# jgkellymit/GENIE-SMEM

Measured on AMD Instinct MI355X. Metric: query-bases/sec SMEM discovery, 100kb ref x 150bp reads; bit-exact SMEM set, higher is better.
Workload: dtype u8/int32 (2-bit packed bases, int32 SA rows; f64 only in the RMI predict)

## Files before the change

### genie-smem_amd/csrc/kernels.hip

```cpp
#include <hip/hip_runtime.h>

#include <algorithm>
#include <cstdio>
#include <cstdlib>
#include <mutex>
#include <string>

#include "genie_internal.h"

namespace genie {

namespace {

constexpr int kWave = 64;

__device__ __forceinline__ int rfl(int v) { return __builtin_amdgcn_readfirstlane(v); }
__device__ __forceinline__ void set_wave_priority(int i)
{
    switch (i & 3) {
    case 0: __builtin_amdgcn_s_setprio(0); break;
    case 1: __builtin_amdgcn_s_setprio(1); break;
    case 2: __builtin_amdgcn_s_setprio(2); break;
    default: __builtin_amdgcn_s_setprio(3); break;
    }
}

__device__ __forceinline__ void scalar_touch_lines(const void *p, uint32_t bytes)
{
    uint32_t d, off;
    asm volatile("s_mov_b32 %[off], 0\n"
                 "1:\n\t"
                 "s_load_dword %[d], %[p], %[off]\n\t"
                 "s_add_u32 %[off], %[off], 64\n\t"
                 "s_cmp_lt_u32 %[off], %[n]\n\t"
                 "s_cbranch_scc1 1b\n\t"
                 "s_waitcnt lgkmcnt(0)"
                 : [d] "=&s"(d), [off] "=&s"(off)
                 : [p] "s"(reinterpret_cast<uint64_t>(p) & ~3ull), [n] "s"(bytes)
                 : "scc", "memory");
}

__device__ __forceinline__ void wave_lds_fence()
{
    __builtin_amdgcn_fence(__ATOMIC_ACQ_REL, "wavefront");
    __builtin_amdgcn_wave_barrier();
}

__device__ __forceinline__ uint64_t funnel(uint64_t w0, uint64_t w1, int sh )
{
    return sh ? (w0 << sh) | (w1 >> (64 - sh)) : w0;
}

__device__ __forceinline__ uint64_t qwin(const uint64_t *qp, int pos)
{
    int i = pos >> 5;
    return funnel(qp[i], qp[i + 1], (pos & 31) * 2);
}

__device__ __forceinline__ uint64_t rwin(const RefRec *ref, int pos)
{
    const ulonglong2 v = *reinterpret_cast<const ulonglong2 *>(ref + (pos >> 5));
    return funnel(v.x, v.y, (pos & 31) * 2);
}

struct QWords {
    const uint64_t *p;
    __device__ __forceinline__ uint64_t win(int pos) const { return qwin(p, pos); }
};
struct QRecs {
    const RefRec *p;
    __device__ __forceinline__ uint64_t win(int pos) const { return rwin(p, pos); }
};
struct QPlain {
    const uint64_t *p;
    __device__ __forceinline__ uint64_t win(int pos) const
    {
        typedef uint64_t u64x2 __attribute__((ext_vector_type(2)));
        typedef u64x2 u64x2_a8 __attribute__((aligned(8)));
        const u64x2 v = *reinterpret_cast<const u64x2_a8 *>(p + (pos >> 5));
        return funnel(v.x, v.y, (pos & 31) * 2);
    }
};

template <class D>
__device__ __forceinline__ uint32_t dir_lb(const DevIndex &ix, const D dir, uint32_t code, int m)
{
    const uint32_t x = code << (2 * (ix.P - m));
    uint32_t v = dir[x];
#pragma unroll
    for (int l = 0; l < GENIE_MAX_DIR_BITS; l++)
        if (l >= m && l < ix.P && ix.padtail[l] == x) v--;
    return v;
}

template <class D>
__device__ __forceinline__ uint32_t dir_ub(const DevIndex &ix, const D dir, uint32_t code, int m)
{
    const uint32_t x = (code + 1) << (2 * (ix.P - m));
    uint32_t v = dir[x];
#pragma unroll
    for (int l = 1; l < GENIE_MAX_DIR_BITS; l++)
        if (l < ix.P && ix.padtail[l] == x) v--;
    return v;
}

struct Cmp {
    int l;
    bool less;
};

template <class Q>
__device__ __forceinline__ Cmp cmp_suffix(const DevIndex &ix, const Q qp, int a, int m, int s, int skip)
{
    const int avail = ix.n - s;
    const int lim = m < avail ? m : avail;
    int l = skip;
    bool less = false;
    bool diff = false;
    while (l < lim) {
        const uint64_t xq = qp.win(a + l), xr = rwin(ix.ref, s + l);
        const uint64_t x = xq ^ xr;
        if (x) {
            l += __clzll((long long)x) >> 1;
            less = xr < xq;
            diff = true;
            break;
        }
        l += 32;
    }
    if (!diff || l >= lim) {
        l = lim;
        less = lim < m;
    }
    return {l, less};
}

template <class Q>
__device__ __forceinline__ Cmp cmp_rec(const DevIndex &ix, const Q qp, int a, int m, const SaRec rec, uint64_t xq)
{
    const int avail = ix.n - rec.s;
    const int lim = m < avail ? m : avail;
    int l = ix.P;
    bool less;
    const uint64_t x = xq ^ rec.key;
    if (x) {
        l += __clzll((long long)x) >> 1;
        less = rec.key < xq;
        if (l >= lim) { l = lim; less = lim < m; }
    } else if (l + 32 >= lim) {
        l = lim;
        less = lim < m;
    } else {
        return cmp_suffix(ix, qp, a, m, rec.s, l + 32);
    }
    return {l, less};
}

__device__ __forceinline__ int pick_probe(int lo, int hi, uint32_t xq32, uint32_t vlo, uint32_t vhi, int step)
{
    const int n = hi - lo;
    if ((step & 1) || n <= 2 || vhi <= vlo) return (lo + hi) >> 1;
    if (xq32 <= vlo) return lo;
    if (xq32 >= vhi) return hi - 1;
    const float f = (float)(xq32 - vlo) / (float)(vhi - vlo);
    int mid = lo + (int)(f * (float)n);
    mid = mid < lo ? lo : (mid > hi - 1 ? hi - 1 : mid);
    return mid;
}

typedef uint32_t nt_u4 __attribute__((ext_vector_type(4)));
typedef nt_u4 nt_u4_unaligned __attribute__((aligned(1)));
__device__ __forceinline__ void store_nt(void *dst, uint4 v)
{
    __builtin_nontemporal_store(nt_u4{v.x, v.y, v.z, v.w}, reinterpret_cast<nt_u4 *>(dst));
}

__device__ __forceinline__ SaRec load_rec(const SaRec *sa, int row)
{
    int4 v = *reinterpret_cast<const int4 *>(sa + row);
    asm volatile("" : "+v"(v.x), "+v"(v.y), "+v"(v.z), "+v"(v.w));
    SaRec r;
    r.s = v.x;
    r.pad = 0;
    r.key = ((uint64_t)(uint32_t)v.w << 32) | (uint32_t)v.z;
    return r;
}

__device__ __forceinline__ bool lut_probe(const DevIndex &ix, uint32_t code, int &lo, int &hi)
{
    uint32_t p = (uint32_t)(((uint64_t)(code * 0x9E3779B1u) * (uint64_t)ix.lut_slots) >> 32);
    for (uint32_t tries = 0; tries < ix.lut_slots; tries++) {
        const int4 v = *reinterpret_cast<const int4 *>(ix.lut + p);
        if (v.y < 0) return false;
        if ((uint32_t)v.x == code) { lo = v.y; hi = v.z; return true; }
        p = p + 1 == ix.lut_slots ? 0 : p + 1;
    }
    return false;
}

__device__ __forceinline__ double rmi_predict(const DevIndex &ix, const RmiModel *leaf, int leaf_cnt, uint32_t code,
                                              int *leaf_idx = nullptr)
{
    const double x = (double)code;
    double p = 0.0;
    int idx = 0;
    for (int l = 0; l < ix.nlev; l++) {
        if (leaf_idx && l == ix.nlev - 1) *leaf_idx = idx;
        double2 m;
        if (leaf && l == ix.nlev - 1 && idx < leaf_cnt) m = *reinterpret_cast<const double2 *>(leaf + idx);
        else m = *reinterpret_cast<const double2 *>(ix.rmi + ix.rmi_off[l] + idx);
        p = __dadd_rn(__dmul_rn(m.x, x), m.y);
        const int scale = ix.rmi_scale[l];
        idx = !(p > 0.0) ? 0 : (p >= (double)scale ? scale - 1 : (int)p);
    }
    return p;
}

__device__ __forceinline__ int kmer_cmp_row(const DevIndex &ix, int r, uint32_t code)
{
    const int s = ix.sa[r].s;
    const int avail = ix.n - s;
    if (avail == 0) return -1;
    const uint64_t w = rwin(ix.ref, s);
    if (avail >= ix.K) {
        const uint32_t rc = (uint32_t)(w >> (64 - 2 * ix.K));
        return rc < code ? -1 : (rc > code ? 1 : 0);
    }
    const uint32_t rc = (uint32_t)(w >> (64 - 2 * avail));
    const uint32_t qc = code >> (2 * (ix.K - avail));
    return rc <= qc ? -1 : 1;
}

__device__ __forceinline__ bool rmi_lookup(const DevIndex &ix, const RmiModel *leaf, uint32_t code, int &lo, int &hi,
                                           double *pred_out)
{
    int leaf_idx = 0;
    const double p = rmi_predict(ix, leaf, 0, code, &leaf_idx);
    if (pred_out) *pred_out = p;
    const int rows = ix.n + 1;
    const int r0 = !(p > 0.0) ? 0 : (p >= (double)rows ? rows - 1 : (int)p);
    int L, R;
    bool fenced = false;
    if (ix.rmi_err) {
        const int e = ix.rmi_err[leaf_idx];
        L = r0 - e < 0 ? 0 : r0 - e;
        R = r0 + e + 1 > rows ? rows : r0 + e + 1;
        int l2 = L, r2 = R;
        while (l2 < r2) {
            const int mid = (l2 + r2) >> 1;
            if (kmer_cmp_row(ix, mid, code) < 0) l2 = mid + 1; else r2 = mid;
        }
        if (l2 < rows && kmer_cmp_row(ix, l2, code) == 0 && (l2 > L || L == 0 || kmer_cmp_row(ix, l2 - 1, code) < 0)) {
            L = R = l2;
            fenced = true;
        }
    }
    if (!fenced) {
    if (kmer_cmp_row(ix, r0, code) < 0) {
        L = r0 + 1;
        R = rows;
        for (int step = 1;; step <<= 1) {
            const int pr = r0 + step;
            if (pr >= rows) break;
            if (kmer_cmp_row(ix, pr, code) < 0) L = pr + 1;
            else { R = pr; break; }
        }
    } else {
        R = r0;
        L = 0;
        for (int step = 1;; step <<= 1) {
            const int pr = r0 - step;
            if (pr < 0) break;
            if (kmer_cmp_row(ix, pr, code) < 0) { L = pr + 1; break; }
            R = pr;
        }
    }
    }
    while (L < R) {
        const int mid = (L + R) >> 1;
        if (kmer_cmp_row(ix, mid, code) < 0) L = mid + 1; else R = mid;
    }
    const int first = L;
    if (first >= rows || kmer_cmp_row(ix, first, code) != 0) { lo = first; hi = first - 1; return false; }
    int a = first, b = rows;
    for (int step = 1;; step <<= 1) {
        const int pr = first + step;
        if (pr >= rows) break;
        if (kmer_cmp_row(ix, pr, code) == 0) a = pr;
        else { b = pr; break; }
    }
    while (b - a > 1) {
        const int mid = (a + b) >> 1;
        if (kmer_cmp_row(ix, mid, code) == 0) a = mid; else b = mid;
    }
    lo = first;
    hi = a;
    return true;
}

template <class Q>
__device__ __forceinline__ int2 sa_interval(const DevIndex &ix, const uint32_t *dir, const Q qp, int a, int m)
{
    if (m == 0) return make_int2(0, ix.n);
    const int P = ix.P;
    const uint64_t w = qp.win(a);
    if (m <= P) {
        const uint32_t code = (uint32_t)(w >> (64 - 2 * m));
        const int lb = (int)dir_lb(ix, dir, code, m), ub = (int)dir_ub(ix, dir, code, m);
        return lb < ub ? make_int2(lb, ub - 1) : make_int2(-1, -1);
    }
    const uint64_t xq = qp.win(a + P);
    int lo, hi, h;
    int known = -1;
    if (ix.P2 && m >= ix.P2) {
        int4 hd = *reinterpret_cast<const int4 *>(ix.dir2 + (uint32_t)(w >> (64 - 2 * ix.P2)));
        asm volatile("" : "+v"(hd.x), "+v"(hd.y), "+v"(hd.z), "+v"(hd.w));
        const uint32_t cnt = (uint32_t)hd.y & ~kHeadShort;
        if (cnt == 0) return make_int2(-1, -1);
        lo = hd.x;
        hi = h = hd.x + (int)cnt;
        const uint64_t key = ((uint64_t)(uint32_t)hd.w << 32) | (uint32_t)hd.z;
        const uint64_t x = xq ^ key;
        if (!((uint32_t)hd.y & kHeadShort) && (x != 0 || m <= P + 32)) {
            const int l = x ? P + (__clzll((long long)x) >> 1) : m;
            if (l >= m) { h = lo; known = lo; }
            else if (key < xq) lo = lo + 1;
            else h = lo;
        }
    } else {
        const uint32_t b = (uint32_t)(w >> (64 - 2 * P));
        lo = (int)dir[b];
        hi = h = (int)dir_ub(ix, dir, b, P);
    }
    uint32_t vlo = 0, vhi = 0xFFFFFFFFu;
    int step = 0;
    while (lo < h) {
        const int mid = pick_probe(lo, h, (uint32_t)(xq >> 32), vlo, vhi, step++);
        const SaRec rec = load_rec(ix.sa, mid);
        const Cmp c = cmp_rec(ix, qp, a, m, rec, xq);
        if (c.less) { lo = mid + 1; vlo = (uint32_t)(rec.key >> 32); }
        else { h = mid; vhi = (uint32_t)(rec.key >> 32); known = c.l >= m ? mid : -1; }
    }
    const int first = lo;
    if (known == first) lo = first + 1;
    h = hi;
    int stepw = 1;
    while (lo < h) {
        int mid = stepw ? lo + stepw - 1 : (lo + h) >> 1;
        if (mid >= h) mid = (lo + h) >> 1;
        if (cmp_rec(ix, qp, a, m, load_rec(ix.sa, mid), xq).l >= m) { lo = mid + 1; stepw = stepw && stepw < (1 << 20) ? stepw << 1 : stepw; }
        else { h = mid; stepw = 0; }
    }
    return first < lo ? make_int2(first, lo - 1) : make_int2(-1, -1);
}

struct WaveScratch {
    uint64_t *qp;
    uint8_t *raw;
};

__host__ __device__ inline int scratch_qp_bytes(int Lmax) { return (((Lmax + 31) / 32 + 2) * 8 + 15) & ~15; }
__host__ __device__ inline int scratch_raw_bytes(int Lmax) { return (Lmax + 15) & ~15; }
__host__ __device__ inline int scratch_bytes(int Lmax) { return scratch_qp_bytes(Lmax) + scratch_raw_bytes(Lmax); }

__device__ __forceinline__ WaveScratch carve(uint8_t *base, int Lmax)
{
    WaveScratch s;
    s.qp = reinterpret_cast<uint64_t *>(base);
    s.raw = base + scratch_qp_bytes(Lmax);
    return s;
}

__device__ __forceinline__ bool load_and_pack(const uint8_t *src, int L, int Lmax, const WaveScratch &ws, int lane)
{
    uint8_t *raw = ws.raw;
    bool bad = false;
    for (int i = lane; i < L; i += kWave) {
        const uint8_t c = src[i];
        bad |= c > 3;
        raw[i] = c;
    }
    wave_lds_fence();
// ... 792 lines not shown
```

### genie-smem_amd/csrc/short_read_kernel.inc

```

template <bool WIDE>
struct ReadTraits {
    typedef uint8_t fwd_t;
    static constexpr int kj_bits = 16, kj_shift = 8;
};
template <>
struct ReadTraits<true> {
    typedef uint16_t fwd_t;
    static constexpr int kj_bits = 32, kj_shift = 16;
};


typedef unsigned short kb_us2 __attribute__((ext_vector_type(2)));
__device__ __forceinline__ uint32_t kb_pk_max(uint32_t a, uint32_t b)
{
    return __builtin_bit_cast(uint32_t, __builtin_elementwise_max(__builtin_bit_cast(kb_us2, a), __builtin_bit_cast(kb_us2, b)));
}

constexpr int kPairHeadWords = 4;

__device__ __forceinline__ int block_exclusive_scan(int v, int &total)
{
    __shared__ int wave_total[16];
    const int lane = threadIdx.x & (kWave - 1), wave = threadIdx.x >> 6;
// ... 25 lines not shown
                                                        uint8_t *__restrict__ counts8, uint8_t *__restrict__ status8)
{
    extern __shared__ __align__(16) uint8_t smem[];
    typedef ReadTraits<false>::fwd_t fwd_t;
    constexpr int kBits = ReadTraits<false>::kj_bits, kShift = ReadTraits<false>::kj_shift, kPer = 64 / kBits;
    const long long r0 = (long long)blockIdx.x * blockDim.x;
    {
        const int rows = (int)(N - r0 < (long long)blockDim.x ? N - r0 : (long long)blockDim.x);
        const uint4 *src = reinterpret_cast<const uint4 *>(reinterpret_cast<const uint8_t *>(fwd_in) + r0 * (long long)fwd_stride);
        uint32_t *dst = reinterpret_cast<uint32_t *>(smem);
        const int ldw = fwd_lds >> 2, upr = fwd_stride >> 4;
        const uint32_t recip = (uint32_t)((0x100000000ull + (uint64_t)upr - 1) / (uint64_t)upr);
        const int units = rows * upr;
        constexpr int kInFlight = 8;
        for (int e0 = threadIdx.x; e0 < units; e0 += kInFlight * blockDim.x) {
            uint4 v[kInFlight];
#pragma unroll
            for (int u = 0; u < kInFlight; u++) {
                const int e = e0 + u * blockDim.x;
                v[u] = e < units ? src[e] : make_uint4(0, 0, 0, 0);
            }
#pragma unroll
            for (int u = 0; u < kInFlight; u++) {
                const int e = e0 + u * blockDim.x;
                if (e < units) {
                    const int row = upr > 1 ? (int)__umulhi((uint32_t)e, recip) : e;
                    const int col = 4 * (e - row * upr);
                    uint32_t *d = dst + row * ldw + col;
                    d[0] = v[u].x;
                    if (col + 1 < ldw) d[1] = v[u].y;
                    if (col + 2 < ldw) d[2] = v[u].z;
                    if (col + 3 < ldw) d[3] = v[u].w;
                }
            }
        }
        __syncthreads();
    }
    const long long r = r0 + threadIdx.x;
    const bool valid = r < N;
    int cnt = 0;
    if (valid) {
        int st = status[r];
        const int L = lens ? lens[r] : fixed_len;
        const fwd_t *fw = reinterpret_cast<const fwd_t *>(smem + threadIdx.x * fwd_lds);
        unsigned long long *out64 = reinterpret_cast<unsigned long long *>(reinterpret_cast<uint8_t *>(kj_out) +
                                                                           r * (long long)kj_stride * (kBits / 8));
        unsigned long long *head64 = reinterpret_cast<unsigned long long *>(head_out + r * (long long)head_stride);
        unsigned long long acc = 0, acc0 = 0;

#define EMIT(kk, jj)                                                          \
        do {                                                                      \
            const int s_ = cnt + 1;                                               \
            const unsigned long long v_ = (unsigned long long)(uint32_t)((kk) | ((jj) << kShift)) << (kBits * (s_ & (kPer - 1))); \
            if (s_ < kPer) acc0 |= v_;                                            \
            else {                                                                \
                acc |= v_;                                                        \
                if ((s_ & (kPer - 1)) == kPer - 1) { (s_ / kPer < kPairHeadWords ? head64 : out64)[s_ / kPer] = acc; acc = 0; } \
            }                                                                     \
            cnt++;                                                                \
        } while (0)

        if (st == GENIE_READ_OK && L > 0) {
            int i = 0, kprev = -1;
            const uint32_t *fw32 = reinterpret_cast<const uint32_t *>(fw);
            while (i < L) {
                const int p0 = kprev + 1;
                const uint32_t i4 = (uint32_t)i * 0x01010101u;
                int sd = p0 >> 2;
                uint32_t x = (fw32[sd] ^ i4) & (~0u << (8 * (p0 & 3)));
                while (x == 0 && sd < (i >> 2)) x = fw32[++sd] ^ i4;
                const int s0 = 4 * sd + ((__ffs((int)x) - 1) >> 3);
                if (x == 0 || s0 > i) { st = GENIE_READ_ABSENT_BASE; break; }
                const uint32_t *pd = fw32 + (s0 >> 2);
                int more = (i >> 2) - (s0 >> 2);
                uint32_t pos = (uint32_t)(s0 >> 2) * 0x04040404u + 0x03020100u;
                uint32_t vb = ~0u << (8 * (s0 & 3));
                const uint32_t vl = ~0u >> (8 * (3 - (i & 3)));
                if (more == 0) vb &= vl;
                uint32_t len4 = (*pd - pos) & vb, pin4 = ~pos & vb;
                uint32_t top0 = __builtin_amdgcn_perm(len4, pin4, 0x05010400u), top1 = __builtin_amdgcn_perm(len4, pin4, 0x07030602u);
                if (more > 0) {
                    while (--more > 0) {
                        pos += 0x04040404u;
                        len4 = *++pd - pos;
                        pin4 = ~pos;
                        top0 = kb_pk_max(top0, __builtin_amdgcn_perm(len4, pin4, 0x05010400u));
                        top1 = kb_pk_max(top1, __builtin_amdgcn_perm(len4, pin4, 0x07030602u));
                    }
                    pos += 0x04040404u;
                    len4 = (*++pd - pos) & vl;
                    pin4 = ~pos & vl;
                    top0 = kb_pk_max(top0, __builtin_amdgcn_perm(len4, pin4, 0x05010400u));
                    top1 = kb_pk_max(top1, __builtin_amdgcn_perm(len4, pin4, 0x07030602u));
                }
                const uint32_t mx = kb_pk_max(top0, top1);
                const uint32_t key = max(mx & 0xFFFFu, mx >> 16);
                const int best = (int)(key >> 8), bk = 255 - (int)(key & 255u);
                if (best == 0) { st = GENIE_READ_ABSENT_BASE; break; }
                if (MODE != GENIE_MODE_BWA || best >= min_len) EMIT(bk, bk + best);
                i = bk + best;
                kprev = bk;
            }
            if (st != GENIE_READ_OK) cnt = 0;
            else {
                if (cnt + 1 >= kPer && ((cnt + 1) & (kPer - 1))) ((cnt + 1) / kPer < kPairHeadWords ? head64 : out64)[(cnt + 1) / kPer] = acc;
                if (cnt > cap) st = GENIE_READ_OVERFLOW;
            }
        }
#undef EMIT
        head64[0] = cnt ? acc0 | (unsigned long long)(uint32_t)cnt : 0ull;
        status[r] = st;
        if (counts8) {
            counts8[r] = (uint8_t)cnt;
            status8[r] = (uint8_t)st;
        }
    }
    if (block_sums) {
        int total;
        const int before = block_exclusive_scan(cnt, total);
        if (valid) counts[r] = before;
        if (threadIdx.x == 0) block_sums[blockIdx.x] = (unsigned long long)total;
    } else if (valid) {
        counts[r] = cnt;
    }
}

template <int G>
__device__ __forceinline__ uint32_t group_max(uint32_t v)
{
    v = max(v, (uint32_t)__builtin_amdgcn_update_dpp(0, (int)v, 0xB1, 0xf, 0xf, true));
    if (G >= 4) v = max(v, (uint32_t)__builtin_amdgcn_update_dpp(0, (int)v, 0x4E, 0xf, 0xf, true));
    if (G >= 8) v = max(v, (uint32_t)__builtin_amdgcn_update_dpp(0, (int)v, 0x141, 0xf, 0xf, true));
    if (G == 16) v = max(v, (uint32_t)__builtin_amdgcn_update_dpp(0, (int)v, 0x140, 0xf, 0xf, true));
    return v;
}

constexpr int kLongWin = 128;
constexpr int kLongRowBytes = 2 * kLongWin + 16;
template <int MODE, int G, int V = 1>
__global__ void __launch_bounds__(256) traverse_long_kernel(const int32_t *__restrict__ lens, long long N, int fixed_len, int min_len,
                                                             const uint8_t *__restrict__ fwd_in, int fwd_stride,
                                                             int32_t *__restrict__ counts, uint32_t *__restrict__ kj_out,
                                                             int kj_stride, int cap, int32_t *__restrict__ status,
                                                             unsigned long long *__restrict__ block_sums)
{
    static_assert((V == 1 && (G == 8 || G == 16)) || (V == 8 && (G == 2 || G == 4)), "lanes per read / positions per lane");
    extern __shared__ __align__(16) uint8_t smem[];
    uint8_t *wrow = smem + (threadIdx.x / G) * kLongRowBytes;
    const int row_chunks = fwd_stride >> 4;
    int wb = -(1 << 20);
    constexpr int kShift = ReadTraits<true>::kj_shift;
    const int lane = threadIdx.x & (kWave - 1), sub = lane & (G - 1);
    const long long r = (long long)blockIdx.x * (blockDim.x / G) + (threadIdx.x / G);
    const bool valid = r < N;
    int st = valid ? status[r] : GENIE_READ_OK;
    const int L = valid ? (lens ? lens[r] : fixed_len) : 0;
    const uint16_t *fw = reinterpret_cast<const uint16_t *>(fwd_in + (valid ? r : 0) * (long long)fwd_stride);
    uint32_t *row = kj_out + (valid ? r : 0) * (long long)kj_stride;
    int i = 0, cnt = 0;
    uint32_t mine = 0;
    bool go = valid && st == GENIE_READ_OK && L > 0;
    int kprev = -1;
    while (__any(go)) {
        uint32_t best = 0;
        int top = i;
        bool more = go;
        if (V == 8) {
            int ctop = i >> 3;
            const uint32_t reach = ((uint32_t)i << 16) | 0xFFFFu;
            bool first = true;
            const int need_lo = (kprev + 1) & ~7;
            const bool fits = go && i - need_lo < kLongWin;
            const bool reload = fits && !(need_lo >= wb && i < wb + kLongWin);
            if (__any(reload)) {
                if (reload) {
                    wb = need_lo;
                    uint4 t[kLongWin / 8 / G];
#pragma unroll
                    for (int u = 0; u < kLongWin / 8 / G; u++) {
                        const int c = (wb >> 3) + sub + G * u;
                        t[u] = c < row_chunks ? *reinterpret_cast<const uint4 *>(fw + 8 * c) : make_uint4(0, 0, 0, 0);
                    }
#pragma unroll
                    for (int u = 0; u < kLongWin / 8 / G; u++) *reinterpret_cast<uint4 *>(wrow + 16 * (sub + G * u)) = t[u];
                }
                wave_lds_fence();
            }
            while (__any(more)) {
                const int c = ctop - sub;
                const bool inb = more && c >= 0;
                uint4 q = make_uint4(0, 0, 0, 0);
                if (inb) {
                    if (fits && 8 * c >= wb) q = *reinterpret_cast<const uint4 *>(wrow + 2 * (8 * c - wb));
                    else q = *reinterpret_cast<const uint4 *>(fw + 8 * c);
                }
                uint32_t qd[4] = {q.x, q.y, q.z, q.w};
                if (first) {
                    const int jmax = (sub == 0) ? (i & 7) : 7;
#pragma unroll
                    for (int d = 0; d < 4; d++) qd[d] &= jmax >= 2 * d + 1 ? 0xFFFFFFFFu : (jmax >= 2 * d ? 0x0000FFFFu : 0u);
                    first = false;
                }
                const uint32_t c0 = (uint32_t)(0xFFFF - 8 * c) - ((uint32_t)(8 * c) << 16);
                uint32_t kmax = 0;
#pragma unroll
                for (int j = 0; j < 8; j++) {
                    const uint32_t vh = (j & 1) ? (qd[j >> 1] & 0xFFFF0000u) : (qd[j >> 1] << 16);
                    const uint32_t key = vh > reach ? vh + (c0 - (uint32_t)j * 0x10001u) : 0u;
                    kmax = max(kmax, key);
                }
                best = max(best, group_max<G>(kmax));
                const bool low = inb && (qd[0] << 16) > reach;
                ctop -= G;
                more = more && ((__ballot(low) >> (lane | (G - 1))) & 1ull);
            }
        }
        while (V == 1 && __any(more)) {
            const int k = top - sub;
            const bool in = more && k > kprev;
            const int v = in ? (int)fw[k] : 0;
            const bool covers = in && v > i;
            const uint32_t key = covers ? ((uint32_t)(v - k) << 16) | (uint32_t)(0xFFFF - k) : 0u;
            best = max(best, group_max<G>(key));
            top -= G;
            more = more && ((__ballot(covers) >> (lane | (G - 1))) & 1ull);
        }
        if (go) {
            const int blen = (int)(best >> 16), bk = 0xFFFF - (int)(best & 0xFFFFu);
            if (blen == 0) { st = GENIE_READ_ABSENT_BASE; go = false; }
            else {
                if (MODE != GENIE_MODE_BWA || blen >= min_len) {
                    const int s_ = cnt + 1;
                    if (sub == (s_ & (G - 1))) mine = (uint32_t)(bk | ((bk + blen) << kShift));
                    if ((s_ & (G - 1)) == G - 1) {
                        const int idx = (s_ & ~(G - 1)) + sub;
                        if (idx > 0) row[idx] = mine;
                    }
                    cnt++;
                }
                kprev = bk;
                i = bk + blen;
                go = i < L;
            }
        }
    }
    if (valid) {
        if (st != GENIE_READ_OK) cnt = 0;
        else {
            const int idx = ((cnt + 1) & ~(G - 1)) + sub;
            if (((cnt + 1) & (G - 1)) != 0 && idx >= 1 && idx <= cnt) row[idx] = mine;
            if (cnt > cap) st = GENIE_READ_OVERFLOW;
        }
        if (sub == 0) {
            row[0] = (uint32_t)cnt;
            status[r] = st;
        }
    }
    if (block_sums) {
        int total;
        const int before = block_exclusive_scan(valid && sub == 0 ? cnt : 0, total);
        if (valid && sub == 0) counts[r] = before;
        if (threadIdx.x == 0) block_sums[blockIdx.x] = (unsigned long long)total;
    } else if (valid && sub == 0) {
        counts[r] = cnt;
    }
}

constexpr int kIvWaves = 8;
constexpr int kIvUnroll = 1;
constexpr int kIvList = 128;

struct RowEscapes {
    unsigned long long *count;
    long long *list;
    long long cap;
};
template <int COUT>
__device__ __forceinline__ void emit_row(void *out, long long idx, int k, int j, int lo, int hi, const RowEscapes &esc)
{
    if (COUT == 0) {
        store_nt(reinterpret_cast<int4 *>(out) + idx, make_uint4((uint32_t)k, (uint32_t)j, (uint32_t)lo, (uint32_t)hi));
        return;
    }
    constexpr uint32_t kTop = COUT == 1 ? 0xFFFFu : 0xFFu;
    uint32_t span = (uint32_t)(hi - lo);
    if (span >= kTop) {
        const unsigned long long slot = atomicAdd(esc.count, 1ull);
        if ((long long)slot < esc.cap) {
            esc.list[2 * slot] = idx;
            esc.list[2 * slot + 1] = hi;
        }
        span = kTop;
    }
    if (COUT == 1) {
        reinterpret_cast<uint2 *>(out)[idx] = make_uint2((uint32_t)k | (uint32_t)j << 8 | span << 16, (uint32_t)lo);
    } else {
        uint16_t *o = reinterpret_cast<uint16_t *>(out) + 3 * idx;
        o[0] = (uint16_t)((uint32_t)k | (uint32_t)j << 8);
        o[1] = (uint16_t)lo;
        o[2] = (uint16_t)(((uint32_t)lo >> 16) | span << 8);
    }
}

template <bool CSR, bool WIDE, bool C16, int COUT = 0>
__global__ void __launch_bounds__(kIvWaves * 64, 8) interval_kernel(DevIndex ix, long long N,
                                                                    const void *__restrict__ kj_in, int kj_stride,
                                                                    const uint8_t *__restrict__ head_in, int head_stride,
                                                                    const RefRec *__restrict__ qp_in, int qp_stride,
                                                                    void *__restrict__ out, int cap,
                                                                    long long *__restrict__ offsets, long long out_cap,
                                                                    const unsigned long long *__restrict__ block_base,
                                                                    const int32_t *__restrict__ before_in_block, int block_shift,
                                                                    RowEscapes esc, int sched)
{
    __shared__ int4 lists[kIvWaves][kIvList];
    typedef typename std::conditional<WIDE, uint32_t, uint16_t>::type kj_t;
    typedef typename std::conditional<WIDE, QRecs, QPlain>::type QIn;
    constexpr int kHeadEntries = kPairHeadWords * 8 / (int)sizeof(kj_t);
    const int lane = threadIdx.x & (kWave - 1);
    const int wave = rfl((int)(threadIdx.x >> 6));
    const int sub = lane & 15;
    const int P2 = ix.P2;
    const __amdgpu_buffer_rsrc_t ov =
        __builtin_amdgcn_make_buffer_rsrc(const_cast<MatchOv16 *>(ix.ov), 0, ix.ov_entries * (int)sizeof(MatchOv16), 0x00020000);
    int4 *list = lists[wave];
    int nlist = 0;
    auto search_list = [&](int o, int n) {
        if (lane < n) {
            const int4 en = list[o + lane];
            const int k = en.w & 0xFFFF, j = (int)((uint32_t)en.w >> 16);
            const QIn qp{reinterpret_cast<decltype(QIn::p)>(qp_in + (long long)en.z * qp_stride)};
            const int2 iv = sa_interval(ix, ix.dir, qp, k, j - k);
            emit_row<COUT>(out, ((long long)en.y << 32) | (uint32_t)en.x, k, j, iv.x, iv.y, esc);
        }
    };
    constexpr int U = kIvUnroll;
    const long long step = (long long)gridDim.x * kIvWaves * 4 * U;
    const bool rotate = !(sched & 1);
    const int round_of_block = (int)(blockIdx.x / (uint32_t)(sched >> 8));
    int it = round_of_block;
    for (long long r0 = ((long long)blockIdx.x * kIvWaves + wave) * 4 * U; r0 < N; r0 += step, it++) {
        if (rotate) set_wave_priority(it);
        long long r[U], base[U];
        int c[U];
        bool more = false;
#pragma unroll
        for (int u = 0; u < U; u++) {
            r[u] = r0 + 4 * u + (lane >> 4);
            const bool have = r[u] < N;
            if (!have) r[u] = 0;
            c[u] = have ? (int)reinterpret_cast<const kj_t *>(head_in + r[u] * (long long)head_stride)[0] : 0;
            base[u] = CSR ? (have ? (long long)block_base[r[u] >> block_shift] + before_in_block[r[u]] : 0) : r[u] * (long long)cap;
            if (CSR && have && sub == 0) {
                if (!COUT) offsets[r[u]] = base[u];
                if (r[u] == N - 1) offsets[COUT ? 0 : N] = base[u] + c[u];
            }
            if (!CSR) c[u] = c[u] < cap ? c[u] : cap;
            more |= c[u] > 0;
        }
        for (int t0 = 0; __any(more); t0 += 16) {
            const int t = t0 + sub;
            uint32_t e[U];
            uint64_t w[U];
            int4 ra[U], rb[U];
            bool act[U];
            more = false;
#pragma unroll
            for (int u = 0; u < U; u++) {
                act[u] = t < c[u] && (!CSR || base[u] + t < out_cap);
                more |= t0 + 16 < c[u];
                const kj_t *row = t + 1 < kHeadEntries ? reinterpret_cast<const kj_t *>(head_in + r[u] * (long long)head_stride)
                                                       : reinterpret_cast<const kj_t *>(kj_in) + r[u] * (long long)kj_stride;
                e[u] = act[u] ? (uint32_t)row[t + 1] : 0u;
            }
#pragma unroll
            for (int u = 0; u < U; u++) {
                const int k = (int)(e[u] & ((1u << ReadTraits<WIDE>::kj_shift) - 1));
                w[u] = act[u] ? QIn{reinterpret_cast<decltype(QIn::p)>(qp_in + r[u] * (long long)qp_stride)}.win(k) : 0ull;
            }
#pragma unroll
            for (int u = 0; u < U; u++) {
                const uint32_t c = (uint32_t)(w[u] >> (64 - 2 * P2));
                const int4 *en = C16 ? reinterpret_cast<const int4 *>(reinterpret_cast<const MatchRec16 *>(ix.mtab) + c)
                                     : reinterpret_cast<const int4 *>(ix.mtab + c);
                ra[u] = make_int4(0, 0, 0, 0);
                rb[u] = make_int4(0, 0, 0, 0);
                if (act[u]) { ra[u] = en[0]; if (!C16) rb[u] = en[1]; }
            }
#pragma unroll
            for (int u = 0; u < U; u++) {
                const int k = (int)(e[u] & ((1u << ReadTraits<WIDE>::kj_shift) - 1)), j = (int)(e[u] >> ReadTraits<WIDE>::kj_shift);
                const int len = j - k;
                const uint32_t meta = (uint32_t)ra[u].x;
                bool fast = false;
                int2 iv = make_int2(-1, -1);
                if (C16) {
                    const uint32_t cnt4 = (meta >> 24) & 15u, nib = meta >> 28, lb = meta & 0xFFFFFFu;
                    if (act[u] && cnt4 == 0) {
                        if (len == (int)nib) { fast = true; iv = make_int2((int)lb, ra[u].y); }
                    } else if (act[u] && (nib & kM16Wide) && cnt4 <= 3u && len >= P2) {
                        const uint32_t xk = (uint32_t)((w[u] << (2 * P2)) >> 32);
                        const int cl = len - P2 < 16 ? len - P2 : 16;
                        const uint32_t km = cl == 0 ? 0u : ~0u << (32 - 2 * cl);
                        const uint32_t bits = (((((uint32_t)ra[u].y ^ xk) & km) == 0 ? 1u : 0u) | ((((uint32_t)ra[u].z ^ xk) & km) == 0 ? 2u : 0u) |
                                               ((((uint32_t)ra[u].w ^ xk) & km) == 0 ? 4u : 0u)) & ((1u << cnt4) - 1u);
                        fast = len <= P2 + 16 || __popc(bits) == 1;
                        if (bits) {
                            const int first = (int)lb + __ffs((int)bits) - 1;
                            iv = make_int2(first, first + __popc(bits) - 1);
                        }
                    } else if (act[u] && (cnt4 == kM16More || !(nib & kM16General)) && len >= P2) {
                        const uint32_t total = cnt4 == kM16More ? 7u + nib : cnt4;
                        const uint32_t xk16 = (uint32_t)((w[u] << (2 * P2)) >> 48);
                        const int cl = len - P2 < 8 ? len - P2 : 8;
                        const uint32_t km16 = cl == 0 ? 0u : (0xFFFFu << (16 - 2 * cl)) & 0xFFFFu;
                        const uint32_t k16[6] = {(uint32_t)ra[u].y & 0xFFFFu, (uint32_t)ra[u].y >> 16, (uint32_t)ra[u].z & 0xFFFFu,
                                                 (uint32_t)ra[u].z >> 16, (uint32_t)ra[u].w & 0xFFFFu, (uint32_t)ra[u].w >> 16};
                        const uint32_t ninl = cnt4 == kM16More ? (uint32_t)kM16Keys - 1u : cnt4;
                        uint32_t bits = 0, xm = 0xFFFFu;
#pragma unroll
                        for (int i = 0; i < kM16Keys; i++) bits |= (((k16[i] ^ xk16) & km16) == 0 && (uint32_t)i < ninl) ? 1u << i : 0u;
                        if (cnt4 == kM16More) mt_ov_scan(ov, k16[5], (int)total - (kM16Keys - 1), xk16, km16, xm, bits);
                        fast = len <= P2 + 8 || __popc(bits) == 1;
                        if (bits) {
                            const int first = (int)lb + __ffs((int)bits) - 1;
                            iv = make_int2(first, first + __popc(bits) - 1);
                        }
                    }
                } else if (act[u] && !(meta & kMatchSlow)) {
                    const uint32_t rows = meta >> 24;
                    if (rows == 0) {
                        if (len == (int)(meta & 0xFFu)) { fast = true; iv = make_int2(ra[u].y, ra[u].z); }
                    } else if (len >= P2) {
                        const uint32_t xk = (uint32_t)((w[u] << (2 * P2)) >> 32);
                        const int cl = len - P2 < 16 ? len - P2 : 16;
                        const uint32_t km = cl == 0 ? 0u : ~0u << (32 - 2 * cl);
                        uint32_t bits = ((((uint32_t)ra[u].z ^ xk) & km) == 0 ? 1u : 0u) | ((((uint32_t)ra[u].w ^ xk) & km) == 0 ? 2u : 0u) |
                                        ((((uint32_t)rb[u].x ^ xk) & km) == 0 ? 4u : 0u) | ((((uint32_t)rb[u].y ^ xk) & km) == 0 ? 8u : 0u) |
                                        ((((uint32_t)rb[u].z ^ xk) & km) == 0 ? 16u : 0u) | ((((uint32_t)rb[u].w ^ xk) & km) == 0 ? 32u : 0u);
                        bits &= (1u << rows) - 1u;
                        fast = len <= P2 + 16 || __popc(bits) == 1;
                        if (bits) {
                            const int first = (int)ra[u].y + __ffs((int)bits) - 1;
                            iv = make_int2(first, first + __popc(bits) - 1);
                        }
                    }
                }
                if (fast) emit_row<COUT>(out, base[u] + t, k, j, iv.x, iv.y, esc);
                const bool general = act[u] && !fast;
                const unsigned long long gb = __ballot(general);
                if (gb) {
                    if (general) {
                        const long long row = base[u] + t;
                        list[nlist + __popcll(gb & ((1ull << lane) - 1ull))] = make_int4((int)(uint32_t)row, (int)(row >> 32), (int)r[u], k | (j << 16));
                    }
                    nlist += __popcll(gb);
                    wave_lds_fence();
                    if (nlist >= 64) {
                        nlist -= 64;
                        search_list(nlist, 64);
                        wave_lds_fence();
                    }
                }
            }
        }
    }
    if (nlist) search_list(0, nlist);
}
```

Measured before the change: 202.7 billion.

## Restructure interval kernel addressing, branchless C16 match eval, and deferred list flush

Rewrites the interval kernel's inner loop to use 32-bit byte offsets from per-row base pointers, which cuts 64-bit address arithmetic and register pressure. The C16 match-table decode becomes a branch-free packed-16-bit comparison in a helper. List flushing now happens at the top of each tile iteration and is drained inside the main loop. The DevIndex is reloaded from kernarg inside search_list so its registers need not stay live. This adds asm barriers and more complex packed logic, and it risks subtle correctness differences in the masking and valid-key handling.

```diff
diff --git a/genie-smem_amd/csrc/kernels.hip b/genie-smem_amd/csrc/kernels.hip
--- a/genie-smem_amd/csrc/kernels.hip
+++ b/genie-smem_amd/csrc/kernels.hip
@@ -70,6 +70,11 @@
 struct QRecs {
     const RefRec *p;
     __device__ __forceinline__ uint64_t win(int pos) const { return rwin(p, pos); }
+    static __device__ __forceinline__ uint64_t win_at(const uint8_t *ubase, uint32_t off, int pos)
+    {
+        const ulonglong2 v = *reinterpret_cast<const ulonglong2 *>(ubase + (off + (uint32_t)(pos >> 5) * 16u));
+        return funnel(v.x, v.y, (pos & 31) * 2);
+    }
 };
 struct QPlain {
     const uint64_t *p;
@@ -78,6 +83,13 @@
         typedef uint64_t u64x2 __attribute__((ext_vector_type(2)));
         typedef u64x2 u64x2_a8 __attribute__((aligned(8)));
         const u64x2 v = *reinterpret_cast<const u64x2_a8 *>(p + (pos >> 5));
+        return funnel(v.x, v.y, (pos & 31) * 2);
+    }
+    static __device__ __forceinline__ uint64_t win_at(const uint8_t *ubase, uint32_t off, int pos)
+    {
+        typedef uint64_t u64x2 __attribute__((ext_vector_type(2)));
+        typedef u64x2 u64x2_a8 __attribute__((aligned(8)));
+        const u64x2 v = *reinterpret_cast<const u64x2_a8 *>(ubase + (off + (uint32_t)(pos >> 5) * 8u));
         return funnel(v.x, v.y, (pos & 31) * 2);
     }
 };
diff --git a/genie-smem_amd/csrc/short_read_kernel.inc b/genie-smem_amd/csrc/short_read_kernel.inc
--- a/genie-smem_amd/csrc/short_read_kernel.inc
+++ b/genie-smem_amd/csrc/short_read_kernel.inc
@@ -351,6 +351,98 @@
     }
 }
 
+__device__ __forceinline__ DevIndex iv_index_afresh()
+{
+    union {
+        DevIndex ix;
+        uint32_t w[sizeof(DevIndex) / 4];
+    } u;
+#if defined(__HIP_DEVICE_COMPILE__)
+    typedef const __attribute__((address_space(4))) uint32_t *KernargWords;
+    KernargWords kp = (KernargWords)__builtin_amdgcn_kernarg_segment_ptr();
+    asm volatile("" : "+s"(kp));
+#pragma unroll
+    for (int i = 0; i < (int)(sizeof(DevIndex) / 4); i++) u.w[i] = kp[i];
+#define IV_GLOBAL(f) u.ix.f = (decltype(u.ix.f))(__attribute__((address_space(1))) std::remove_reference<decltype(*u.ix.f)>::type *)reinterpret_cast<uintptr_t>(u.ix.f)
+    IV_GLOBAL(sa); IV_GLOBAL(ref); IV_GLOBAL(dir); IV_GLOBAL(lut); IV_GLOBAL(rmi); IV_GLOBAL(dir2); IV_GLOBAL(rmi_err); IV_GLOBAL(mtab); IV_GLOBAL(ov);
+#undef IV_GLOBAL
+#endif
+    return u.ix;
+}
+
+template <class T>
+__device__ __forceinline__ T iv_load(const uint8_t *ubase, uint32_t off)
+{
+    asm volatile("" : "+v"(off));
+    return *reinterpret_cast<const T *>(ubase + off);
+}
+template <class T>
+__device__ __forceinline__ void iv_store(void *ubase, uint32_t off, T v)
+{
+    asm volatile("" : "+v"(off));
+    *reinterpret_cast<T *>(reinterpret_cast<uint8_t *>(ubase) + off) = v;
+}
+
+__device__ __forceinline__ uint32_t iv_pk_min(uint32_t a, uint32_t b)
+{
+    return __builtin_bit_cast(uint32_t, __builtin_elementwise_min(__builtin_bit_cast(kb_us2, a), __builtin_bit_cast(kb_us2, b)));
+}
+__device__ __forceinline__ uint32_t iv_ctz(uint32_t x) { return x ? (uint32_t)__builtin_ctz(x) : 32u; }
+
+__device__ __forceinline__ uint32_t iv_ov_bits(const __amdgpu_buffer_rsrc_t ov, uint32_t blk, int nov, uint32_t xk16, uint32_t km16)
+{
+    uint32_t off = blk << 4;
+    asm volatile("" : "+v"(off));
+    uint32_t xm = 0xFFFFu, bits = 0;
+    mt_ov_scan(ov, off >> 4, nov, xk16, km16, xm, bits);
+    return bits;
+}
+
+struct IvHit {
+    int lo, hi;
+    bool fast;
+};
+__device__ __forceinline__ IvHit iv_eval16(const __amdgpu_buffer_rsrc_t ov, const int4 en, uint64_t wq, int len, int P2, bool act)
+{
+    const uint32_t meta = (uint32_t)en.x, cnt4 = (meta >> 24) & 15u, nib = meta >> 28, lb = meta & 0xFFFFFFu;
+    const bool wide = (nib & kM16Wide) && cnt4 >= 1u && cnt4 <= 3u;
+    const bool more = cnt4 == kM16More;
+    const bool keyed = act && len >= P2 && cnt4 != 0 && (wide || more || !(nib & kM16General));
+    const int kw = wide ? 16 : 8;
+    int cl = len - P2;
+    cl = cl < kw ? cl : kw;
+    cl = cl > 0 ? cl : 0;
+    const uint32_t kmw = (uint32_t)(~0ull << (32 - 2 * cl));
+    const uint32_t km = wide ? kmw : kmw | kmw >> 16;
+    const uint32_t xk = (uint32_t)((wq << (2 * P2)) >> 32);
+    const uint32_t xx = wide ? xk : __builtin_amdgcn_perm(xk, xk, 0x03020302u);
+    const uint32_t d1 = ((uint32_t)en.y ^ xx) & km, d2 = ((uint32_t)en.z ^ xx) & km, d3 = ((uint32_t)en.w ^ xx) & km;
+    uint32_t one = 0x00010001u;
+    asm("" : "+s"(one));
+    const uint32_t differ = iv_pk_min(d1, one) | iv_pk_min(d2, one) << 1 | iv_pk_min(d3, one) << 2;
+    const uint32_t ninl = more ? (uint32_t)kM16Keys - 1u : cnt4;
+    const uint32_t valid = wide ? (1u << cnt4) - 1u : ((1u << ((ninl + 1u) >> 1)) - 1u) | ((1u << (ninl >> 1)) - 1u) << 16;
+    uint32_t agree = ~differ & 0x00070007u;
+    agree = (wide ? agree & agree >> 16 : agree) & valid;
+    if (!keyed) agree = 0;
+    uint32_t ovb = 0;
+    if (more && keyed) ovb = iv_ov_bits(ov, (uint32_t)en.w >> 16, (int)nib + 2, xk >> 16, km & 0xFFFFu);
+    const int cnt = __popc(agree) + __popc(ovb);
+    uint32_t first = min(iv_ctz(agree & 0xFFFFu) << (wide ? 0 : 1), 2u * iv_ctz(agree >> 16) + 1u);
+    first = min(first, iv_ctz(ovb));
+    const int lo = (int)(lb + first);
+    IvHit h;
+    h.fast = keyed && (len <= P2 + kw || cnt == 1);
+    h.lo = cnt ? lo : -1;
+    h.hi = cnt ? lo + cnt - 1 : -1;
+    if (cnt4 == 0) {
+        h.fast = act && len == (int)nib;
+        h.lo = (int)lb;
+        h.hi = en.y;
+    }
+    return h;
+}
+
 template <bool CSR, bool WIDE, bool C16, int COUT = 0>
 __global__ void __launch_bounds__(kIvWaves * 64, 8) interval_kernel(DevIndex ix, long long N,
                                                                     const void *__restrict__ kj_in, int kj_stride,
@@ -363,12 +455,13 @@
                                                                     RowEscapes esc, int sched)
 {
     __shared__ int4 lists[kIvWaves][kIvList];
+    static_assert(63 + 64 * kIvUnroll <= kIvList, "the list takes one iteration's rows on top of what a flush leaves");
     typedef typename std::conditional<WIDE, uint32_t, uint16_t>::type kj_t;
     typedef typename std::conditional<WIDE, QRecs, QPlain>::type QIn;
     constexpr int kHeadEntries = kPairHeadWords * 8 / (int)sizeof(kj_t);
     const int lane = threadIdx.x & (kWave - 1);
     const int wave = rfl((int)(threadIdx.x >> 6));
-    const int sub = lane & 15;
+    const int sub = lane & 15, g4 = lane >> 4;
     const int P2 = ix.P2;
     const __amdgpu_buffer_rsrc_t ov =
         __builtin_amdgcn_make_buffer_rsrc(const_cast<MatchOv16 *>(ix.ov), 0, ix.ov_entries * (int)sizeof(MatchOv16), 0x00020000);
@@ -376,38 +469,65 @@
     int nlist = 0;
     auto search_list = [&](int o, int n) {
         if (lane < n) {
+            const DevIndex ixs = iv_index_afresh();
             const int4 en = list[o + lane];
             const int k = en.w & 0xFFFF, j = (int)((uint32_t)en.w >> 16);
             const QIn qp{reinterpret_cast<decltype(QIn::p)>(qp_in + (long long)en.z * qp_stride)};
-            const int2 iv = sa_interval(ix, ix.dir, qp, k, j - k);
+            const int2 iv = sa_interval(ixs, ixs.dir, qp, k, j - k);
             emit_row<COUT>(out, ((long long)en.y << 32) | (uint32_t)en.x, k, j, iv.x, iv.y, esc);
         }
     };
     constexpr int U = kIvUnroll;
-    const long long step = (long long)gridDim.x * kIvWaves * 4 * U;
-    const bool rotate = !(sched & 1);
+    const uint32_t step = gridDim.x * (uint32_t)(kIvWaves * 4 * U);
     const int round_of_block = (int)(blockIdx.x / (uint32_t)(sched >> 8));
-    int it = round_of_block;
-    for (long long r0 = ((long long)blockIdx.x * kIvWaves + wave) * 4 * U; r0 < N; r0 += step, it++) {
-        if (rotate) set_wave_priority(it);
-        long long r[U], base[U];
+    int it = (sched & 1) ? -1 : round_of_block;
+    const uint32_t head_o = (uint32_t)(g4 * head_stride);
+    const uint32_t head_e = head_o + (uint32_t)(1 + sub) * (uint32_t)sizeof(kj_t);
+    const uint32_t kj_e = (uint32_t)(g4 * kj_stride + 1 + sub) * (uint32_t)sizeof(kj_t);
+    const uint32_t qp_o = (uint32_t)(g4 * qp_stride) * (uint32_t)sizeof(RefRec);
+    for (long long r0 = ((long long)blockIdx.x * kIvWaves + wave) * 4 * U; r0 < N || nlist > 0; r0 += step) {
+        if (it >= 0) {
+            set_wave_priority(it);
+            it = (it + 1) & 0xFFFF;
+        }
+        const bool drain = r0 >= N;
+        const uint8_t *hb[U], *kb[U], *qb[U];
+        long long base[U];
         int c[U];
         bool more = false;
 #pragma unroll
         for (int u = 0; u < U; u++) {
-            r[u] = r0 + 4 * u + (lane >> 4);
-            const bool have = r[u] < N;
-            if (!have) r[u] = 0;
-            c[u] = have ? (int)reinterpret_cast<const kj_t *>(head_in + r[u] * (long long)head_stride)[0] : 0;
-            base[u] = CSR ? (have ? (long long)block_base[r[u] >> block_shift] + before_in_block[r[u]] : 0) : r[u] * (long long)cap;
-            if (CSR && have && sub == 0) {
-                if (!COUT) offsets[r[u]] = base[u];
-                if (r[u] == N - 1) offsets[COUT ? 0 : N] = base[u] + c[u];
-            }
-            if (!CSR) c[u] = c[u] < cap ? c[u] : cap;
+            const long long ru = r0 + 4 * u;
+            const long long left = N - ru;
+            const int nh = left >= 4 ? 4 : (left > 0 ? (int)left : 0);
+            const bool have = g4 < nh;
+            hb[u] = head_in + (unsigned long long)ru * (uint32_t)head_stride;
+            kb[u] = reinterpret_cast<const uint8_t *>(reinterpret_cast<const kj_t *>(kj_in) + (unsigned long long)ru * (uint32_t)kj_stride);
+            qb[u] = reinterpret_cast<const uint8_t *>(qp_in + (unsigned long long)ru * (uint32_t)qp_stride);
+            c[u] = have ? (int)iv_load<kj_t>(hb[u], head_o) : 0;
+            if (CSR) {
+                const long long bb = nh > 0 ? (long long)block_base[ru >> block_shift] : 0;
+                base[u] = have ? bb + iv_load<int32_t>(reinterpret_cast<const uint8_t *>(before_in_block + ru), (uint32_t)g4 * 4u) : 0;
+                int first_of_16 = sub;
+                asm volatile("" : "+v"(first_of_16));
+                if (have && first_of_16 == 0) {
+                    if (!COUT) iv_store<long long>(offsets + ru, (uint32_t)g4 * 8u, base[u]);
+                    if (left <= 4 && g4 == nh - 1) offsets[COUT ? 0 : N] = base[u] + c[u];
+                }
+            } else {
+                base[u] = ru * (long long)cap + g4 * cap;
+                c[u] = c[u] < cap ? c[u] : cap;
+            }
             more |= c[u] > 0;
         }
-        for (int t0 = 0; __any(more); t0 += 16) {
+        for (int t0 = 0;; t0 += 16) {
+            if (nlist >= 64 || (drain && nlist > 0)) {
+                const int n = nlist < 64 ? nlist : 64;
+                nlist -= n;
+                search_list(nlist, n);
+                wave_lds_fence();
+            }
+            if (!__any(more)) break;
             const int t = t0 + sub;
             uint32_t e[U];
             uint64_t w[U];
@@ -418,23 +538,26 @@
             for (int u = 0; u < U; u++) {
                 act[u] = t < c[u] && (!CSR || base[u] + t < out_cap);
                 more |= t0 + 16 < c[u];
-                const kj_t *row = t + 1 < kHeadEntries ? reinterpret_cast<const kj_t *>(head_in + r[u] * (long long)head_stride)
-                                                       : reinterpret_cast<const kj_t *>(kj_in) + r[u] * (long long)kj_stride;
-                e[u] = act[u] ? (uint32_t)row[t + 1] : 0u;
+                const bool in_head = t + 1 < kHeadEntries;
+                e[u] = 0u;
+                if (act[u] && in_head) e[u] = (uint32_t)iv_load<kj_t>(hb[u], head_e + (uint32_t)t0 * (uint32_t)sizeof(kj_t));
+                if (act[u] && !in_head) e[u] = (uint32_t)iv_load<kj_t>(kb[u], kj_e + (uint32_t)t0 * (uint32_t)sizeof(kj_t));
             }
 #pragma unroll
             for (int u = 0; u < U; u++) {
                 const int k = (int)(e[u] & ((1u << ReadTraits<WIDE>::kj_shift) - 1));
-                w[u] = act[u] ? QIn{reinterpret_cast<decltype(QIn::p)>(qp_in + r[u] * (long long)qp_stride)}.win(k) : 0ull;
+                w[u] = act[u] ? QIn::win_at(qb[u], qp_o, k) : 0ull;
             }
 #pragma unroll
             for (int u = 0; u < U; u++) {
                 const uint32_t c = (uint32_t)(w[u] >> (64 - 2 * P2));
-                const int4 *en = C16 ? reinterpret_cast<const int4 *>(reinterpret_cast<const MatchRec16 *>(ix.mtab) + c)
-                                     : reinterpret_cast<const int4 *>(ix.mtab + c);
+                const uint8_t *tab = reinterpret_cast<const uint8_t *>(ix.mtab);
                 ra[u] = make_int4(0, 0, 0, 0);
                 rb[u] = make_int4(0, 0, 0, 0);
-                if (act[u]) { ra[u] = en[0]; if (!C16) rb[u] = en[1]; }
+                if (act[u]) {
+                    ra[u] = iv_load<int4>(tab, c << (C16 ? 4 : 5));
+                    if (!C16) rb[u] = iv_load<int4>(tab, (c << 5) + 16u);
+                }
             }
 #pragma unroll
             for (int u = 0; u < U; u++) {
@@ -444,38 +567,9 @@
                 bool fast = false;
                 int2 iv = make_int2(-1, -1);
                 if (C16) {
-                    const uint32_t cnt4 = (meta >> 24) & 15u, nib = meta >> 28, lb = meta & 0xFFFFFFu;
-                    if (act[u] && cnt4 == 0) {
-                        if (len == (int)nib) { fast = true; iv = make_int2((int)lb, ra[u].y); }
-                    } else if (act[u] && (nib & kM16Wide) && cnt4 <= 3u && len >= P2) {
-                        const uint32_t xk = (uint32_t)((w[u] << (2 * P2)) >> 32);
-                        const int cl = len - P2 < 16 ? len - P2 : 16;
-                        const uint32_t km = cl == 0 ? 0u : ~0u << (32 - 2 * cl);
-                        const uint32_t bits = (((((uint32_t)ra[u].y ^ xk) & km) == 0 ? 1u : 0u) | ((((uint32_t)ra[u].z ^ xk) & km) == 0 ? 2u : 0u) |
-                                               ((((uint32_t)ra[u].w ^ xk) & km) == 0 ? 4u : 0u)) & ((1u << cnt4) - 1u);
-                        fast = len <= P2 + 16 || __popc(bits) == 1;
-                        if (bits) {
-                            const int first = (int)lb + __ffs((int)bits) - 1;
-                            iv = make_int2(first, first + __popc(bits) - 1);
-                        }
-                    } else if (act[u] && (cnt4 == kM16More || !(nib & kM16General)) && len >= P2) {
-                        const uint32_t total = cnt4 == kM16More ? 7u + nib : cnt4;
-                        const uint32_t xk16 = (uint32_t)((w[u] << (2 * P2)) >> 48);
-                        const int cl = len - P2 < 8 ? len - P2 : 8;
-                        const uint32_t km16 = cl == 0 ? 0u : (0xFFFFu << (16 - 2 * cl)) & 0xFFFFu;
-                        const uint32_t k16[6] = {(uint32_t)ra[u].y & 0xFFFFu, (uint32_t)ra[u].y >> 16, (uint32_t)ra[u].z & 0xFFFFu,
-                                                 (uint32_t)ra[u].z >> 16, (uint32_t)ra[u].w & 0xFFFFu, (uint32_t)ra[u].w >> 16};
-                        const uint32_t ninl = cnt4 == kM16More ? (uint32_t)kM16Keys - 1u : cnt4;
-                        uint32_t bits = 0, xm = 0xFFFFu;
-#pragma unroll
-                        for (int i = 0; i < kM16Keys; i++) bits |= (((k16[i] ^ xk16) & km16) == 0 && (uint32_t)i < ninl) ? 1u << i : 0u;
-                        if (cnt4 == kM16More) mt_ov_scan(ov, k16[5], (int)total - (kM16Keys - 1), xk16, km16, xm, bits);
-                        fast = len <= P2 + 8 || __popc(bits) == 1;
-                        if (bits) {
-                            const int first = (int)lb + __ffs((int)bits) - 1;
-                            iv = make_int2(first, first + __popc(bits) - 1);
-                        }
-                    }
+                    const IvHit h = iv_eval16(ov, ra[u], w[u], len, P2, act[u]);
+                    fast = h.fast;
+                    iv = make_int2(h.lo, h.hi);
                 } else if (act[u] && !(meta & kMatchSlow)) {
                     const uint32_t rows = meta >> 24;
                     if (rows == 0) {
@@ -501,18 +595,13 @@
                 if (gb) {
                     if (general) {
                         const long long row = base[u] + t;
-                        list[nlist + __popcll(gb & ((1ull << lane) - 1ull))] = make_int4((int)(uint32_t)row, (int)(row >> 32), (int)r[u], k | (j << 16));
+                        list[nlist + __popcll(gb & ((1ull << lane) - 1ull))] =
+                            make_int4((int)(uint32_t)row, (int)(row >> 32), (int)(r0 + 4 * u) + g4, k | (j << 16));
                     }
                     nlist += __popcll(gb);
                     wave_lds_fence();
-                    if (nlist >= 64) {
-                        nlist -= 64;
-                        search_list(nlist, 64);
-                        wave_lds_fence();
-                    }
-                }
-            }
-        }
-    }
-    if (nlist) search_list(0, nlist);
-}
+                }
+            }
+        }
+    }
+}
```

Result: no change. 201.1 billion (-0.8%).
